# SitaoLuan/When-Do-GNNs-Help

Measured on AMD Instinct MI355X. Metric: aggregation edges/sec (whole job; + %HBM roofline of the SpMM kernel), higher is better.
Workload: dtype f32; 1 GPU; synthetic homophily sweep (data_synthesis/4000-equivalent): 10 h-levels x 5 seeds = 50 graphs/GPU/step, N=2000 nodes, k=10, F=500 fp32, C=5; step = batched D^-1(A+I)X aggregation + edge/label stati...; parallelism=independent sweep shards x1 (no data-path collective; job-table broadcast + r...

## Files before the change

include/wdg.h:

```cpp
#ifndef WDG_H
#define WDG_H

#include <stddef.h>
#include <stdint.h>

#ifdef __cplusplus
extern "C" {
#endif

typedef void *wdg_stream_t;

#define WDG_OK 0
#define WDG_ERR_INVALID (-1)
#define WDG_ERR_LAUNCH (-2)
#define WDG_ERR_WORKSPACE (-3)
#define WDG_ERR_UNSUPPORTED (-4)

int wdg_version(void);
const char *wdg_last_error(void);
int wdg_device_cus(void);

#define WDG_COO_SYMMETRISE 1
#define WDG_COO_BINARISE 2
#define WDG_COO_ADD_SELF_LOOPS 4
// ... 97 lines not shown
    const int32_t *rowptr;
    const int32_t *col;
    const float *val;
    int32_t *q_perm, *q_ext, *q_rows;
    int32_t *q_col;
    float *q_val;
    void *workspace;
    int32_t n_rows, n_cols;
} wdg_sell16_job;
int wdg_csr_to_sell16_count_batched(const wdg_sell16_job *jobs_dev, int32_t n_jobs, int32_t max_rows, int32_t max_cols,
                                    wdg_stream_t stream);
int wdg_csr_to_sell16_fill_batched(const wdg_sell16_job *jobs_dev, int32_t n_jobs, int32_t max_rows, int32_t max_cols,
                                   wdg_stream_t stream);

size_t wdg_csr_band_plan_workspace_bytes(int32_t N);
int32_t wdg_csr_band_perm_len(int32_t N);
int wdg_csr_band_plan(const int32_t *rowptr, int32_t N, int32_t *band_perm, int32_t *band_cuts, void *workspace,
                      size_t workspace_bytes, wdg_stream_t stream);
int wdg_csr_band_plan_hub(const int32_t *rowptr, int32_t N, int32_t hub_len, int32_t *band_perm, int32_t *band_cuts, void *workspace,
                          size_t workspace_bytes, wdg_stream_t stream);

int32_t wdg_spmm_narrow_col_bytes(int32_t n_feat, int32_t x_is_bf16, int32_t has_col_scale);
int32_t wdg_spmm_narrow_parts(int32_t n_cols, int32_t col_bytes);
size_t wdg_spmm_narrow_workspace_bytes(int32_t n_rows, int32_t n_cols);
int wdg_spmm_narrow_plan(const int32_t *rowptr, const int32_t *col, int32_t N, int32_t n_cols, int32_t parts, int32_t *part_ptr,
                         wdg_stream_t stream);
int wdg_spmm_narrow_f32(const wdg_spmm_job *job_host, const int32_t *part_ptr, void *workspace, size_t workspace_bytes,
                        wdg_stream_t stream);
int wdg_spmm_narrow_bf16(const wdg_spmm_job *job_host, const int32_t *part_ptr, void *workspace, size_t workspace_bytes,
                         wdg_stream_t stream);

int wdg_spmm_narrow_batched_f32(const wdg_spmm_job *jobs_dev, int32_t n_jobs, int32_t max_rows, int32_t max_feat, int flags,
                                wdg_stream_t stream);

typedef struct wdg_spmm_item {
    int32_t first_job, n_jobs;
    int32_t unit_begin, unit_end;
    int32_t flags, reserved;
} wdg_spmm_item;
int wdg_spmm_quad_batched_f32(const wdg_spmm_job *jobs_dev, int32_t n_jobs, const wdg_spmm_item *items_dev,
                              const int32_t *seg_ptr_dev, int32_t n_segments, int32_t max_cols, int32_t max_feat, int flags,
                              wdg_stream_t stream);
int wdg_spmm_quad_batched_clocked_f32(const wdg_spmm_job *jobs_dev, int32_t n_jobs, const wdg_spmm_item *items_dev,
                                      const int32_t *seg_ptr_dev, int32_t n_segments, int32_t max_cols, int32_t max_feat,
                                      int flags, uint64_t *wg_clock_dev, wdg_stream_t stream);
int32_t wdg_spmm_quad_workgroups(int32_t n_segments, int32_t max_feat, int flags);
int wdg_debug_clock(uint64_t *out_dev, wdg_stream_t stream);

int wdg_edge_label_stats(const int32_t *rowptr, const int32_t *col, const int32_t *labels, int32_t N, int32_t C,
                         int64_t *totals, int32_t *row_nnz, int32_t *row_nnz_noself, int32_t *row_match_noself,
                         int64_t *compat, int64_t *classdeg, wdg_stream_t stream);

typedef struct wdg_stats_job {
    const int32_t *rowptr;
    const int32_t *col;
    const int32_t *labels;
    int64_t *totals;
    int64_t *compat;
    int64_t *classdeg;
    int32_t *row_nnz, *row_nnz_noself, *row_match_noself;
    int32_t n_rows, n_classes;
} wdg_stats_job;
int wdg_edge_label_stats_batched(const wdg_stats_job *jobs_dev, int32_t n_jobs, int32_t max_rows, int32_t max_classes,
                                 wdg_stream_t stream);

int wdg_sweep_scalars_f32(const int64_t *totals, const int32_t *rows, const int64_t *compat, const int64_t *classdeg,
// ... 207 lines not shown
```

when-do-gnns-help_amd/_lib.py:

```python
import ctypes
import os

os.environ.setdefault("GPU_MAX_HW_QUEUES", "8")

import torch

_HERE = os.path.dirname(os.path.abspath(__file__))
LIB_PATH = os.environ.get("WDG_LIB_PATH") or os.path.join(_HERE, "lib", "libwdg_hip.so")

c_void_p, c_int, c_int32, c_int64, c_size_t = (ctypes.c_void_p, ctypes.c_int, ctypes.c_int32, ctypes.c_int64,
                                               ctypes.c_size_t)
c_uint32 = ctypes.c_uint32


class WdgError(RuntimeError):
    pass


class SpmmJob(ctypes.Structure):
    _fields_ = [("rowptr", c_void_p), ("col", c_void_p), ("val", c_void_p), ("row_scale", c_void_p),
                ("col_scale", c_void_p), ("X", c_void_p), ("Y", c_void_p), ("ldx", c_int64), ("ldy", c_int64),
                ("n_rows", c_int32), ("n_cols", c_int32), ("n_feat", c_int32), ("reserved", c_int32),
                ("q_ext", c_void_p), ("q_col", c_void_p), ("q_val", c_void_p), ("q_perm", c_void_p), ("q_rows", c_void_p),
                ("q_block_cols", c_int32), ("q_n_blocks", c_int32), ("q_n_entries", c_int32), ("q_flags", c_int32),
# ... 30 lines not shown
    "wdg_csr_to_sell16_fill_batched": (c_int, [c_void_p, c_int32, c_int32, c_int32, c_void_p]),
    "wdg_dense_to_csr_count": (c_int, [c_void_p, c_int64, c_int32, c_int32, c_void_p, c_void_p, c_size_t, c_void_p]),
    "wdg_dense_to_csr_fill": (c_int, [c_void_p, c_int64, c_int32, c_int32, c_void_p, c_void_p, c_void_p, c_void_p]),
    "wdg_scan_workspace_bytes": (c_size_t, [c_int64]),
    "wdg_degree_norm": (c_int, [c_void_p, c_void_p, c_int32, c_int, c_int, c_void_p, c_void_p, c_void_p, c_void_p,
                                c_void_p]),
    "wdg_normalise_values": (c_int, [c_void_p, c_void_p, c_void_p, c_int32, c_int, c_int, c_void_p, c_void_p,
                                     c_void_p, c_void_p]),
    "wdg_row_l1_normalise_f32": (c_int, [c_void_p, c_int64, c_void_p, c_int64, c_int32, c_int32, c_int, c_void_p]),
    "wdg_unpack_bits_f32": (c_int, [c_void_p, c_int64, c_int32, c_int32, c_int, c_void_p, c_int64, c_void_p]),
    "wdg_spmm_csr_f32": (c_int, [ctypes.POINTER(SpmmJob), c_void_p]),
    "wdg_spmm_csr_bf16": (c_int, [ctypes.POINTER(SpmmJob), c_void_p]),
    "wdg_spmm_batched_f32": (c_int, [c_void_p, c_int32, c_int32, c_int32, c_int32, c_int, c_void_p]),
    "wdg_spmm_plan": (c_int, [c_int32, c_int32, c_int32, c_int32, c_int, ctypes.POINTER(c_int), ctypes.POINTER(c_int)]),
    "wdg_sell16_block_cols": (c_int32, [c_int32]),
    "wdg_sell16_row_bytes": (c_int32, [c_int32]),
    "wdg_sell16_workspace_bytes": (c_size_t, [c_int32, c_int32]),
    "wdg_sell16_max_entries": (c_int64, [c_int32]),
    "wdg_csr_to_sell16_count": (c_int, [c_void_p, c_void_p, c_int32, c_int32, c_void_p, c_void_p, c_void_p, c_void_p, c_size_t,
                                        c_void_p]),
    "wdg_csr_to_sell16_fill": (c_int, [c_void_p, c_void_p, c_void_p, c_int32, c_int32, c_void_p, c_void_p, c_int32, c_void_p,
                                       c_void_p, c_void_p]),
    "wdg_csr_band_plan_workspace_bytes": (c_size_t, [c_int32]),
    "wdg_csr_band_perm_len": (c_int32, [c_int32]),
    "wdg_csr_band_plan": (c_int, [c_void_p, c_int32, c_void_p, c_void_p, c_void_p, c_size_t, c_void_p]),
    "wdg_csr_band_plan_hub": (c_int, [c_void_p, c_int32, c_int32, c_void_p, c_void_p, c_void_p, c_size_t, c_void_p]),
    "wdg_spmm_narrow_col_bytes": (c_int32, [c_int32, c_int32, c_int32]),
    "wdg_spmm_narrow_parts": (c_int32, [c_int32, c_int32]),
    "wdg_spmm_narrow_workspace_bytes": (c_size_t, [c_int32, c_int32]),
    "wdg_spmm_narrow_plan": (c_int, [c_void_p, c_void_p, c_int32, c_int32, c_int32, c_void_p, c_void_p]),
    "wdg_spmm_narrow_f32": (c_int, [c_void_p, c_void_p, c_void_p, c_size_t, c_void_p]),
    "wdg_spmm_narrow_bf16": (c_int, [c_void_p, c_void_p, c_void_p, c_size_t, c_void_p]),
    "wdg_spmm_narrow_batched_f32": (c_int, [c_void_p, c_int32, c_int32, c_int32, c_int, c_void_p]),
    "wdg_spmm_quad_batched_clocked_f32": (c_int, [c_void_p, c_int32, c_void_p, c_void_p, c_int32, c_int32, c_int32, c_int, c_void_p,
                                                  c_void_p]),
    "wdg_spmm_quad_workgroups": (c_int32, [c_int32, c_int32, c_int]),
    "wdg_debug_clock": (c_int, [c_void_p, c_void_p]),
    "wdg_spmm_quad_batched_f32": (c_int, [c_void_p, c_int32, c_void_p, c_void_p, c_int32, c_int32, c_int32, c_int,
                                          c_void_p]),
    "wdg_edge_label_stats": (c_int, [c_void_p, c_void_p, c_void_p, c_int32, c_int32, c_void_p, c_void_p, c_void_p,
                                     c_void_p, c_void_p, c_void_p, c_void_p]),
    "wdg_edge_label_stats_batched": (c_int, [c_void_p, c_int32, c_int32, c_int32, c_void_p]),
    "wdg_sweep_scalars_f32": (c_int, [c_void_p, c_void_p, c_void_p, c_void_p, c_void_p, c_void_p, c_void_p, c_int32, c_int32, c_int32,
                                      c_void_p, c_void_p]),
    "wdg_edge_cosine_f32": (c_int, [c_void_p, c_void_p, c_void_p, c_int64, c_void_p, c_int64, c_int32, c_int32, c_int,
                                    c_void_p, c_void_p]),
    "wdg_las_workspace_bytes": (c_size_t, [c_int32, c_int32, c_int32]),
    "wdg_las_f32": (c_int, [c_void_p, c_int64, c_void_p, c_void_p, c_int32, c_int32, c_int32, c_void_p, c_void_p,
                            c_void_p, c_size_t, c_void_p]),
    "wdg_gemm_f32": (c_int, [c_void_p, c_int64, c_void_p, c_int64, c_int, c_void_p, c_int, c_void_p, c_int64,
                             c_int32, c_int32, c_int32, c_void_p]),
    "wdg_gemm_skinny_f32": (c_int, [c_void_p, c_int64, c_void_p, c_int64, c_void_p, c_int, c_void_p, c_int64, c_int32, c_int32, c_int32,
                                    c_void_p]),
    "wdg_gemm_splitk_plan": (c_int32, [c_int32, c_int32, c_int32]),
    "wdg_gemm_splitk_workspace_bytes": (c_size_t, [c_int32, c_int32, c_int32]),
    "wdg_gemm_splitk_f32": (c_int, [c_void_p, c_int64, c_void_p, c_int64, c_void_p, c_int, c_void_p, c_int64, c_int32, c_int32, c_int32,
                                    c_int32, c_void_p, c_size_t, c_void_p]),
    "wdg_gemm_batched_f32": (c_int, [c_void_p, c_int32, c_int32, c_int32, c_void_p]),
    "wdg_gemm_batched_flags_f32": (c_int, [c_void_p, c_int32, c_int32, c_int32, c_int32, c_uint32, c_void_p]),
    "wdg_mlp2_batched_f32": (c_int, [c_void_p, c_int32, c_int32, c_int32, c_int32, c_int32, c_void_p]),
    "wdg_mlp2_batched_flags_f32": (c_int, [c_void_p, c_int32, c_int32, c_int32, c_int32, c_int32, c_uint32, c_void_p]),
    "wdg_las_batched_f32": (c_int, [c_void_p, c_int32, c_int32, c_int32, c_int32, c_void_p]),
    "wdg_las_fused_eligible": (c_int, [c_int32, c_int32, c_int32]),
    "wdg_gram_map_batched_f32": (c_int, [c_void_p, c_int32, c_int32, c_void_p]),
    "wdg_gram_map_batched_flags_f32": (c_int, [c_void_p, c_int32, c_int32, c_uint32, c_void_p]),
    "wdg_transpose_batched_f32": (c_int, [c_void_p, c_int32, c_int32, c_int32, c_void_p]),
# ... 116 lines not shown
```

when-do-gnns-help_amd/aggregate.py:

```python
import ctypes
import os

import numpy as np
import torch

from . import _lib
from ._lib import c_void_p, check, lib, require_gpu, stream_handle
from ._rt import *
from ._rt import _dev, _h2d, _ld, _ptr, _table
from ._lib import SpmmItem, SpmmJob
from .graphs import CsrGraph, quad_disabled

ABLATE_BITS = 0


NARROW_MIN_ENTRIES = int(os.environ.get("WDG_NARROW_MIN_ENTRIES", 1 << 15))


def _fill_job(job, g, x, y, row_scale, col_scale, use_values=True, band=False):
    job.rowptr, job.col = g.rowptr.data_ptr(), g.col.data_ptr()
    job.val = g.val.data_ptr() if (use_values and g.val is not None and not g.unit_values) else 0
    job.row_scale = 0 if row_scale is None else row_scale.data_ptr()
    job.col_scale = 0 if col_scale is None else col_scale.data_ptr()
    job.X, job.Y = x.data_ptr(), y.data_ptr()
    if isinstance(y, Tiled):
        if y.cols != x.shape[1] or y.shape[0] != g.n_rows:
            raise ValueError("spmm: a tiled Y must hold exactly the product's rows and columns")
        job.ldx, job.ldy, job.y_group_stride = _ld(x), y.ld, y.group_stride
    else:
        job.ldx, job.ldy, job.y_group_stride = _ld(x), _ld(y), 0
    job.n_rows, job.n_cols, job.n_feat = g.n_rows, g.n_cols, x.shape[1]
    job.reserved = ABLATE_BITS
    wants_val = bool(job.val)
    q = g.quad
    if q and (not wants_val or q["val"] is not None):
        job.q_ext, job.q_col, job.q_perm = q["ext"].data_ptr(), q["col"].data_ptr(), q["perm"].data_ptr()
        job.q_rows = q["rows"].data_ptr()
        job.q_val = q["val"].data_ptr() if (wants_val and q["val"] is not None) else 0
        job.q_block_cols, job.q_n_blocks = q["block_cols"], q["n_blocks"]
        job.q_n_entries, job.q_flags = q["n_entries"], (1 if q["split"] else 0) | (2 if q["half"] else 0) | (4 if isinstance(x, Transposed) else 0)
    else:
        job.q_ext = job.q_col = job.q_val = job.q_perm = job.q_rows = 0
        job.q_block_cols = job.q_n_blocks = job.q_n_entries = job.q_flags = 0
    if band and g.band:
        job.band_perm, job.band_cuts = g.band["perm"].data_ptr(), g.band["cuts"].data_ptr()
        job.band_n_hub = g.band.get("n_hub", -1)
        job.q_ext = job.q_col = job.q_val = job.q_perm = job.q_rows = 0
        job.q_block_cols = job.q_n_blocks = job.q_n_entries = job.q_flags = 0
# ... 217 lines not shown
            if x.dtype != torch.float32 or x.stride(1) != 1:
                raise ValueError("SpmmBatch: X must be fp32 with unit inner stride")
        feats = {e[1].shape[1] for e in entries}
        need_ld = 8 if max(feats, default=0) > 4 else 4
        self.narrow = (len(entries) > 0 and max(feats) <= 8 and os.environ.get("WDG_SPMM_NARROW", "1") != "0"
                       and all(e[1].data_ptr() % 16 == 0 and _ld(e[1]) % 4 == 0 and _ld(e[1]) >= need_ld for e in entries))
        self.quad = (len(entries) > 0 and not self.narrow and not quad_disabled() and min(feats) >= 8
                     and all(e[0].ensure_quad() for e in entries)
                     and all((not (e[5] and e[0].val is not None)) or e[0].quad["val"] is not None for e in entries)
                     and len({e[0].quad["half"] for e in entries}) == 1)
        order = sorted(range(len(entries)), key=lambda i: -entries[i][0].nnz)
        if os.environ.get("WDG_SPMM_ORDER") == "0":
            order = list(range(len(entries)))
        if self.quad:
            groups = _sharing_groups(entries)
            groups.sort(key=lambda grp: -sum(entries[i][0].nnz for i in grp))
            order = [i for grp in groups for i in sorted(grp, key=lambda i: -entries[i][0].nnz)]
        if any(isinstance(e[2], Tiled) for e in entries) and not self.quad:
            raise ValueError("SpmmBatch: a tiled Y needs the quad-row kernel (SELL-16 copies, F >= 8)")
        if any(isinstance(e[1], Transposed) for e in entries) and not self.quad:
            raise ValueError("SpmmBatch: a transposed X needs the quad-row kernel (SELL-16 copies, F >= 8)")
        for job, (g, x, y, rs, cs, uv) in zip(arr, (entries[i] for i in order)):
            _fill_job(job, g, x, y, rs, cs, uv)
            any_val = any_val or bool(job.val)
            dma_ok = dma_ok and _dma_ok(job)
            self.max_rows, self.max_cols = max(self.max_rows, g.n_rows), max(self.max_cols, g.n_cols)
            self.max_feat = max(self.max_feat, x.shape[1])
        self.n_jobs = len(entries)
        self.table = _table(arr)
        self.edges = sum(e[0].nnz for e in entries)
        self.flags = (SPMM_ANY_VAL if any_val else 0) | (SPMM_DMA_OK if dma_ok else 0)
        if any(e[4] is not None for e in entries):
            self.flags |= SPMM_ANY_COL_SCALE
        if self.quad:
            if all(_y_span(e[2], e[0].n_rows) < (1 << 30) and e[0].quad["chunks"] < (1 << 22) - 2 and e[0].quad["split"] for e in entries):
                self.flags |= SPMM_SMALL_OFFSETS
            if entries[0][0].quad["half"]:
                self.flags |= SPMM_HALF_SLAB
            self.order = order
            self._set_segments(None)
            if os.environ.get("WDG_QUAD_VERIFY", "0") not in ("", "0"):
                self.verify()

    def verify(self, tol=1e-5):
        if not self.quad:
            return
        self.launch()
        torch.cuda.synchronize()
        for i, (g, x, y, rs, cs, uv) in enumerate(self.keep):
            got = y.rowmajor() if isinstance(y, Tiled) else y.clone()
            ref = torch.empty((g.n_rows, x.shape[1]), dtype=torch.float32, device=y.device)
            xv = x.t.t().contiguous() if isinstance(x, Transposed) else x
            job = _fill_job(SpmmJob(), g, xv, ref, rs, cs, uv)
            job.q_ext = job.q_col = job.q_val = job.q_perm = job.q_rows = 0
            job.q_block_cols = job.q_n_blocks = job.q_n_entries = job.q_flags = 0
            check(lib.wdg_spmm_csr_f32(ctypes.byref(job), stream_handle()), "wdg_spmm_csr_f32")
            torch.cuda.synchronize()
            err = float((got[:, :x.shape[1]] - ref).abs().max()) if ref.numel() else 0.0
            scale = max(float(ref.abs().max()) if ref.numel() else 0.0, 1e-30)
            if not err <= tol * scale:
                raise RuntimeError(f"WDG_QUAD_VERIFY: job {i} of the quad-row table differs from the CSR kernel by {err:.3e} "
                                   f"(largest entry {scale:.3e})")

    def _set_segments(self, phase_ns, shares=None):
        dev = self.table.device
        items, seg_ptr, self.n_segments = _quad_segments(self.keep, self.order, self.max_feat, max(lib.wdg_device_cus(), 8), phase_ns, shares)
        iarr = (SpmmItem * max(len(items), 1))()
        for it, (fj, nj, ub, ue) in zip(iarr, items):
            it.first_job, it.n_jobs, it.unit_begin, it.unit_end = fj, nj, ub, ue
        self.items = _h2d(torch.frombuffer(bytearray(bytes(iarr)), dtype=torch.uint8), dev)
        self.seg_ptr = _h2d(np.asarray(seg_ptr, np.int32), dev)
        self.n_items = len(items)
        self.items_host, self.seg_ptr_host, self.phase_ns, self.shares = items, seg_ptr, phase_ns, shares

    def segment_spans(self, clock):
# ... 8 lines not shown
            return None
        best = None
        for ph in candidates:
            self._set_segments(ph)
            self.launch()
            e0, e1 = torch.cuda.Event(enable_timing=True), torch.cuda.Event(enable_timing=True)
            torch.cuda.synchronize()
            e0.record()
            for _ in range(launches):
                self.launch()
            e1.record()
            torch.cuda.synchronize()
            t = e0.elapsed_time(e1) / launches
            if best is None or t < best[0]:
                best = (t, ph)
        self._set_segments(best[1])
        self.tuned = best
        return best

    def new_clock(self):
        n = int(lib.wdg_spmm_quad_workgroups(self.n_segments, self.max_feat, self.flags))
        return torch.zeros(2 * n, dtype=torch.int64, device=self.table.device)

    n_launches = 0

    def launch(self, clock=None):
        self.n_launches += 1
        if clock is not None and self.quad:
            check(lib.wdg_spmm_quad_batched_clocked_f32(_ptr(self.table), self.n_jobs, _ptr(self.items), _ptr(self.seg_ptr),
                                                        self.n_segments, self.max_cols, self.max_feat, self.flags, _ptr(clock),
                                                        stream_handle()), "wdg_spmm_quad_batched_clocked_f32")
            return
        if self.narrow:
            check(lib.wdg_spmm_narrow_batched_f32(_ptr(self.table), self.n_jobs, self.max_rows, self.max_feat, self.flags,
                                                  stream_handle()), "wdg_spmm_narrow_batched_f32")
            return
        if self.quad:
            check(lib.wdg_spmm_quad_batched_f32(_ptr(self.table), self.n_jobs, _ptr(self.items), _ptr(self.seg_ptr),
                                                self.n_segments, self.max_cols, self.max_feat, self.flags, stream_handle()),
                  "wdg_spmm_quad_batched_f32")
            return
        check(lib.wdg_spmm_batched_f32(_ptr(self.table), self.n_jobs, self.max_rows, self.max_cols, self.max_feat,
                                       self.flags, stream_handle()), "wdg_spmm_batched_f32")

    def plan(self):
        if self.narrow:
            return 6, 16, 256
        if self.quad:
            return 5, 16, 1024
        return spmm_plan(self.max_rows, self.max_cols, self.max_feat, self.n_jobs, self.flags)

    def kernel_name(self):
        fam, slab, threads = self.plan()
        val = "true" if self.flags & SPMM_ANY_VAL else "false"
        return {0: f"spmm_slab_kernel<{slab},{threads},float>", 1: "spmm_gather_kernel",
                5: f"spmm_quad_kernel<float,{val},{2 if self.flags & SPMM_HALF_SLAB else (1 if self.max_cols > 2528 else 0)}>",
                6: "spmm_narrow_batched_kernel"}.get(fam, f"family {fam}")


def spmm_plan(n_rows, n_cols, n_feat, n_jobs=1, flags=0):
    slab, threads = ctypes.c_int(0), ctypes.c_int(0)
    fam = lib.wdg_spmm_plan(n_jobs, n_rows, n_cols, n_feat, flags, ctypes.byref(slab), ctypes.byref(threads))
    return fam, slab.value, threads.value
```

when-do-gnns-help_amd/csrc/spmm_narrow.hip:

```cpp
#include <algorithm>

#include "wdg_common.h"

namespace {
using namespace wdg;

constexpr int N_THREADS = 256;
constexpr int N_WAVES = N_THREADS / kWave;

typedef unsigned short bf16_t;

template <typename TIN>
__device__ __forceinline__ float n_f32(TIN v);
template <>
__device__ __forceinline__ float n_f32<float>(float v) { return v; }
template <>
__device__ __forceinline__ float n_f32<bf16_t>(bf16_t v) { return __uint_as_float(static_cast<unsigned>(v) << 16); }

template <typename TIN>
__global__ __launch_bounds__(256) void narrow_pack(const TIN *__restrict__ X, int64_t ldx, const float *__restrict__ cs, int n_cols,
                                                   int F, float *__restrict__ T) {
    const int64_t i = static_cast<int64_t>(blockIdx.x) * 256 + threadIdx.x;
    if (i >= static_cast<int64_t>(n_cols) * 8) return;
    const int c = static_cast<int>(i >> 3), f = static_cast<int>(i & 7);
// ... 4 lines not shown

template <typename TIN>
__global__ __launch_bounds__(256) void narrow_pack4(const TIN *__restrict__ X, int64_t ldx, const float *__restrict__ cs, int n_cols,
                                                    int F, float *__restrict__ T) {
    const int64_t i = static_cast<int64_t>(blockIdx.x) * 256 + threadIdx.x;
    if (i >= static_cast<int64_t>(n_cols) * 4) return;
    const int c = static_cast<int>(i >> 2), f = static_cast<int>(i & 3);
    float v = 0.f;
    if (f < F) v = n_f32<TIN>(X[static_cast<int64_t>(c) * ldx + f]) * (cs ? cs[c] : 1.f);
    T[i] = v;
}
__global__ __launch_bounds__(256) void narrow_pack_bf16x8(const bf16_t *__restrict__ X, int64_t ldx, int n_cols, int F,
                                                          bf16_t *__restrict__ T) {
    const int64_t i = static_cast<int64_t>(blockIdx.x) * 256 + threadIdx.x;
    if (i >= static_cast<int64_t>(n_cols) * 8) return;
    const int c = static_cast<int>(i >> 3), f = static_cast<int>(i & 7);
    T[i] = f < F ? X[static_cast<int64_t>(c) * ldx + f] : static_cast<bf16_t>(0);
}

enum { TABLE_F32X8 = 0, TABLE_F32X4 = 1, TABLE_BF16X8 = 2 };

struct Acc8 {
    float v[8];
};

__device__ __forceinline__ void narrow_unpack_bf16(const f32x4_t raw, f32x4_t &lo, f32x4_t &hi) {
    const unsigned w0 = __float_as_uint(raw[0]), w1 = __float_as_uint(raw[1]), w2 = __float_as_uint(raw[2]), w3 = __float_as_uint(raw[3]);
    lo[0] = __uint_as_float(w0 << 16); lo[1] = __uint_as_float(w0 & 0xffff0000u);
    lo[2] = __uint_as_float(w1 << 16); lo[3] = __uint_as_float(w1 & 0xffff0000u);
    hi[0] = __uint_as_float(w2 << 16); hi[1] = __uint_as_float(w2 & 0xffff0000u);
    hi[2] = __uint_as_float(w3 << 16); hi[3] = __uint_as_float(w3 & 0xffff0000u);
}

template <int G, bool HAS_W, bool WIDE = true, bool BF16 = false>
__device__ __forceinline__ Acc8 narrow_sweep(global_ptr<const int32_t> col, global_ptr<const float> val,
                                             global_ptr<const f32x4_t> T, int b, int e, int sub, int64_t ldq = 2,
                                             global_ptr<const float> cs = nullptr) {
    Acc8 a;
#pragma unroll
    for (int f = 0; f < 8; ++f) a.v[f] = 0.f;
    const f32x4_t zero = {0.f, 0.f, 0.f, 0.f};
    int k = b + sub;
    for (; k + 3 * G < e; k += 4 * G) {
        int idx[4];
        float w[4];
        f32x4_t lo[4], hi[4];
#pragma unroll
        for (int u = 0; u < 4; ++u) idx[u] = col[k + u * G];
#pragma unroll
        for (int u = 0; u < 4; ++u) {
            lo[u] = T[ldq * static_cast<int64_t>(idx[u])];
            hi[u] = (WIDE && !BF16) ? T[ldq * static_cast<int64_t>(idx[u]) + 1] : zero;
            w[u] = 1.f;
            if (HAS_W) w[u] = (val ? val[k + u * G] : 1.f) * (cs ? cs[idx[u]] : 1.f);
        }
#pragma unroll
        for (int u = 0; u < 4; ++u) {
            if (BF16) narrow_unpack_bf16(lo[u], lo[u], hi[u]);
#pragma unroll
            for (int f = 0; f < 4; ++f) {
                a.v[f] = HAS_W ? __builtin_fmaf(w[u], lo[u][f], a.v[f]) : a.v[f] + lo[u][f];
                if (WIDE) a.v[4 + f] = HAS_W ? __builtin_fmaf(w[u], hi[u][f], a.v[4 + f]) : a.v[4 + f] + hi[u][f];
            }
        }
    }
    for (; k < e; k += G) {
        const int idx = col[k];
        f32x4_t lo = T[ldq * static_cast<int64_t>(idx)], hi = (WIDE && !BF16) ? T[ldq * static_cast<int64_t>(idx) + 1] : zero;
        if (BF16) narrow_unpack_bf16(lo, lo, hi);
        float w = 1.f;
        if (HAS_W) w = (val ? val[k] : 1.f) * (cs ? cs[idx] : 1.f);
#pragma unroll
        for (int f = 0; f < 4; ++f) {
            a.v[f] = HAS_W ? __builtin_fmaf(w, lo[f], a.v[f]) : a.v[f] + lo[f];
            if (WIDE) a.v[4 + f] = HAS_W ? __builtin_fmaf(w, hi[f], a.v[4 + f]) : a.v[4 + f] + hi[f];
        }
    }
    return a;
}

__device__ __forceinline__ float narrow_reduce16(const Acc8 &a, int lane) {
    float h4[4], h2[2];
    const bool b3 = lane & 8, b2 = lane & 4, b1 = lane & 2;
#pragma unroll
    for (int i = 0; i < 4; ++i) {
        const float keep = b3 ? a.v[4 + i] : a.v[i], send = b3 ? a.v[i] : a.v[4 + i];
        h4[i] = keep + __shfl_xor(send, 8);
    }
#pragma unroll
    for (int i = 0; i < 2; ++i) {
        const float keep = b2 ? h4[2 + i] : h4[i], send = b2 ? h4[i] : h4[2 + i];
        h2[i] = keep + __shfl_xor(send, 4);
    }
    const float keep = b1 ? h2[1] : h2[0], send = b1 ? h2[0] : h2[1];
    const float h1 = keep + __shfl_xor(send, 2);
    return h1 + __shfl_xor(h1, 1);
}

__device__ __forceinline__ float narrow_reduce64(Acc8 a, int lane) {
#pragma unroll
    for (int f = 0; f < 8; ++f) a.v[f] += __shfl_xor(a.v[f], 32);
// ... 65 lines not shown
        int b = 0, e = 0;
        if (live) bounds(row, b, e);
        const float total = narrow_reduce16(narrow_sweep<16, HAS_VAL, WIDE, BF16>(col, val, T, b, e, lane & 15, LDQ), lane);
        if (live && !(lane & 1) && feat < n_out) out[static_cast<int64_t>(row) * ldo + feat] = total * scale_of(row);
    }
}

__global__ __launch_bounds__(256) void narrow_plan_kernel(const int32_t *__restrict__ rowptr, const int32_t *__restrict__ col, int N,
                                                          int part_cols, int parts, int32_t *__restrict__ part_ptr) {
    const int64_t i = static_cast<int64_t>(blockIdx.x) * 256 + threadIdx.x;
    if (i >= static_cast<int64_t>(N) * (parts - 1)) return;
    const int row = static_cast<int>(i / (parts - 1)), p = static_cast<int>(i % (parts - 1)) + 1;
    int lo = rowptr[row], hi = rowptr[row + 1];
    const int key = p * part_cols;
    while (lo < hi) {
        const int mid = (lo + hi) >> 1;
        if (col[mid] < key) lo = mid + 1;
        else hi = mid;
    }
    part_ptr[i] = lo;
}

__global__ __launch_bounds__(256) void narrow_combine(const float *__restrict__ P, int N, int parts, int F, const float *__restrict__ rs,
                                                      float *__restrict__ Y, int64_t ldy) {
    const int64_t i = static_cast<int64_t>(blockIdx.x) * 256 + threadIdx.x;
    if (i >= static_cast<int64_t>(N) * 8) return;
    const int row = static_cast<int>(i >> 3), f = static_cast<int>(i & 7);
    if (f >= F) return;
    float sum = P[i];
    for (int p = 1; p < parts; ++p) sum += P[static_cast<int64_t>(p) * N * 8 + i];
    Y[static_cast<int64_t>(row) * ldy + f] = sum * (rs ? rs[row] : 1.f);
}

template <bool HAS_W, bool WIDE>
__global__ __launch_bounds__(N_THREADS) void spmm_narrow_batched_kernel(const wdg_spmm_job *__restrict__ jobs, int blocks_per_job) {
    const int job_id = blockIdx.x / blocks_per_job, rb = blockIdx.x % blocks_per_job;
    const desc_ptr<wdg_spmm_job> job = (desc_ptr<wdg_spmm_job>)(jobs + job_id);
    const int N = job->n_rows, F = job->n_feat;
    const int lane = threadIdx.x & 63;
    const int row = rb * 16 + (threadIdx.x >> 4);
    if (rb * 16 >= N) return;
    const global_ptr<const int32_t> rowptr = to_global(job->rowptr), col = to_global(job->col);
    const global_ptr<const float> val = to_global(job->val), rs = to_global(job->row_scale), cs = to_global(job->col_scale);
    const global_ptr<const f32x4_t> X = (global_ptr<const f32x4_t>)to_global(static_cast<const float *>(job->X));
    const bool live = row < N;
    const int b = live ? rowptr[row] : 0, e = live ? rowptr[row + 1] : 0;
    const float total = narrow_reduce16(narrow_sweep<16, HAS_W, WIDE>(col, val, X, b, e, lane & 15, job->ldx / 4, cs), lane);
    const int feat = (lane >> 1) & 7;
    if (live && !(lane & 1) && feat < F) to_global(job->Y)[static_cast<int64_t>(row) * job->ldy + feat] = total * (rs ? rs[row] : 1.f);
}

constexpr int64_t N_PART_BYTES = 3 << 20;

}

extern "C" {

int32_t wdg_spmm_narrow_col_bytes(int32_t n_feat, int32_t x_is_bf16, int32_t has_col_scale) {
    return (n_feat <= 4 || (x_is_bf16 && !has_col_scale)) ? 16 : 32;
}

int32_t wdg_spmm_narrow_parts(int32_t n_cols, int32_t col_bytes) {
    if (const char *s = getenv("WDG_NARROW_PARTS")) {
        const int v = atoi(s);
        if (v == 1 || v == 2 || v == 4 || v == 8) return v;
    }
    int parts = 1;
    while (parts < 8 && static_cast<int64_t>(n_cols) * col_bytes > N_PART_BYTES * parts) parts <<= 1;
    return parts;
}

size_t wdg_spmm_narrow_workspace_bytes(int32_t n_rows, int32_t n_cols) {
    const int parts = wdg_spmm_narrow_parts(n_cols, 32);
    return static_cast<size_t>(n_cols > 0 ? n_cols : 0) * 32 + (parts > 1 ? static_cast<size_t>(parts) * (n_rows > 0 ? n_rows : 0) * 32 : 0) + 512;
}

int wdg_spmm_narrow_plan(const int32_t *rowptr, const int32_t *col, int32_t N, int32_t n_cols, int32_t parts, int32_t *part_ptr,
                         wdg_stream_t stream) {
    WDG_REQUIRE(N >= 0 && n_cols >= 0, "spmm_narrow_plan: negative size");
    WDG_REQUIRE(parts == 1 || parts == 2 || parts == 4 || parts == 8, "spmm_narrow_plan: parts must be 1, 2, 4 or 8");
    if (parts == 1 || N == 0) return WDG_OK;
    WDG_REQUIRE(rowptr && col && part_ptr, "spmm_narrow_plan: null array");
// ... 37 lines not shown
        else
            hipLaunchKernelGGL(narrow_pack<float>, dim3(blocks), dim3(256), 0, st, static_cast<const float *>(j->X), j->ldx, j->col_scale, j->n_cols, j->n_feat, T);
    }
    const int cus = std::max(wdg_device_cus(), 8);
    const int per_cu = 8;
    const dim3 grid(static_cast<unsigned>(cus / kXcds * kXcds * per_cu));
#define WDG_NARROW_LAUNCH(V, TB) hipLaunchKernelGGL((spmm_narrow_kernel<V, TB>), grid, dim3(N_THREADS), 0, st, *j, T, part_ptr, parts, P)
    if (j->val) {
        if (table == TABLE_F32X8) WDG_NARROW_LAUNCH(true, TABLE_F32X8);
        else if (table == TABLE_F32X4) WDG_NARROW_LAUNCH(true, TABLE_F32X4);
        else WDG_NARROW_LAUNCH(true, TABLE_BF16X8);
    } else {
        if (table == TABLE_F32X8) WDG_NARROW_LAUNCH(false, TABLE_F32X8);
        else if (table == TABLE_F32X4) WDG_NARROW_LAUNCH(false, TABLE_F32X4);
        else WDG_NARROW_LAUNCH(false, TABLE_BF16X8);
    }
#undef WDG_NARROW_LAUNCH
    if (parts > 1) {
        const unsigned blocks = static_cast<unsigned>(wdg::ceil_div(static_cast<int64_t>(j->n_rows) * 8, 256));
        hipLaunchKernelGGL(narrow_combine, dim3(blocks), dim3(256), 0, st, P, j->n_rows, parts, j->n_feat, j->row_scale, j->Y, j->ldy);
    }
    return wdg::check_launch("spmm_narrow_kernel");
}

int wdg_spmm_narrow_f32(const wdg_spmm_job *job_host, const int32_t *part_ptr, void *workspace, size_t workspace_bytes,
                        wdg_stream_t stream) {
    return narrow_launch(job_host, false, part_ptr, workspace, workspace_bytes, stream);
}
int wdg_spmm_narrow_bf16(const wdg_spmm_job *job_host, const int32_t *part_ptr, void *workspace, size_t workspace_bytes,
                         wdg_stream_t stream) {
    return narrow_launch(job_host, true, part_ptr, workspace, workspace_bytes, stream);
}

int wdg_spmm_narrow_batched_f32(const wdg_spmm_job *jobs_dev, int32_t n_jobs, int32_t max_rows, int32_t max_feat, int flags,
                                wdg_stream_t stream) {
    WDG_REQUIRE(n_jobs >= 0 && max_rows >= 0 && max_feat >= 0, "spmm_narrow_batched: negative size");
    if (n_jobs == 0 || max_rows == 0 || max_feat == 0) return WDG_OK;
    WDG_REQUIRE(jobs_dev != nullptr, "spmm_narrow_batched: null job table");
    if (max_feat > 8) return wdg::fail(WDG_ERR_UNSUPPORTED, "spmm_narrow_batched: more than 8 features");
    const int blocks_per_job = static_cast<int>(wdg::ceil_div(max_rows, 16));
    WDG_REQUIRE(static_cast<int64_t>(blocks_per_job) * n_jobs < (1ll << 31), "spmm_narrow_batched: grid too large");
    const dim3 grid(static_cast<unsigned>(blocks_per_job) * n_jobs);
    hipStream_t st = wdg::as_stream(stream);
    const bool has_w = (flags & (WDG_SPMM_ANY_VAL | WDG_SPMM_ANY_COL_SCALE)) != 0, wide = max_feat > 4;
    if (has_w) {
        if (wide) hipLaunchKernelGGL((spmm_narrow_batched_kernel<true, true>), grid, dim3(N_THREADS), 0, st, jobs_dev, blocks_per_job);
        else hipLaunchKernelGGL((spmm_narrow_batched_kernel<true, false>), grid, dim3(N_THREADS), 0, st, jobs_dev, blocks_per_job);
    } else {
        if (wide) hipLaunchKernelGGL((spmm_narrow_batched_kernel<false, true>), grid, dim3(N_THREADS), 0, st, jobs_dev, blocks_per_job);
        else hipLaunchKernelGGL((spmm_narrow_batched_kernel<false, false>), grid, dim3(N_THREADS), 0, st, jobs_dev, blocks_per_job);
    }
    return wdg::check_launch("spmm_narrow_batched_kernel");
}

}
```

when-do-gnns-help_amd/ops.py:

```python
from ._lib import check, lib, require_gpu, stream_handle
from ._rt import (
    ACT_NONE, ACT_RELU, COO_ADD_SELF_LOOPS, COO_BINARISE, COO_DROP_SELF_LOOPS, COO_KEEP_DUPLICATES, COO_SYMMETRISE,
    GEMM_A_VEC4, NORM_RW, NORM_SYM, PREC_F32, PREC_F64, SPMM_ANY_COL_SCALE, SPMM_ANY_VAL, SPMM_DMA_OK,
    SPMM_HALF_SLAB, SPMM_SMALL_OFFSETS, Tiled, Transposed, _dev, _h2d, _H2D_MAX_BYTES, _ld, _PinnedArena, _ptr, _table,
)
from .graphs import (
    CsrGraph, degree_norm, GraphBatch, normalise_values, quad_disabled, row_l1_normalise, unpack_bits,
    _host_pack_coo,
)
from .aggregate import (
    QUAD_MULTI_ITEM_SU, spmm, spmm_plan, SpmmBatch, _dma_ok, _fill_job, _QUAD_COST_NS,
    _QUAD_COST_W, _quad_cut, _quad_segments, _quad_unit_cost, _quad_unit_costs, _sharing_groups,
)
from .stats import (
    edge_cosine, edge_label_stats, las, LasBatch, StatsBatch,
)
from .gemm import (
    gemm, gemm_skinny, GemmBatch, Mlp2Batch,
)
from .kernel_regression import (
    deflation_enabled, EdgeGramBatch, GnbBatch, GramBatch, kr_split_sizes, KrBatch, KrSets, PropagatedGram, RowRepBatch, SvmBatch, _KR_JOB_DTYPE,
)
```

Measured before the change: 18.16 billion edges/s.

## Stage narrow SpMM source rows in LDS with software-pipelined row extents

Adds an LDS-staged route for the batched narrow SpMM. Each workgroup of 512 threads copies the whole narrow source matrix (and column scales) of its job into up to 128 KiB of dynamic LDS, then sweeps a contiguous slice of rows. It also prefetches row extents and the first four column indices two steps ahead. The host chooses a parts-per-job count from CU count, rows and the edge-to-column ratio. This replaces scattered global gathers with LDS reads, at the cost of a redundant per-workgroup staging load and occupancy limited to one large block per CU.

```diff
diff --git a/include/wdg.h b/include/wdg.h
--- a/include/wdg.h
+++ b/include/wdg.h
@@ -153,6 +153,12 @@
 
 int wdg_spmm_narrow_batched_f32(const wdg_spmm_job *jobs_dev, int32_t n_jobs, int32_t max_rows, int32_t max_feat, int flags,
                                 wdg_stream_t stream);
+#define WDG_NARROW_IN_PLACE 0
+#define WDG_NARROW_LDS_512 1
+#define WDG_NARROW_LDS_1024 2
+int32_t wdg_spmm_narrow_lds_bytes(int32_t max_cols, int32_t max_feat, int flags);
+int wdg_spmm_narrow_batched_routed_f32(const wdg_spmm_job *jobs_dev, int32_t n_jobs, int32_t max_rows, int32_t max_cols,
+                                       int32_t max_feat, int flags, int32_t route, int32_t parts, wdg_stream_t stream);
 
 typedef struct wdg_spmm_item {
     int32_t first_job, n_jobs;
diff --git a/when-do-gnns-help_amd/_lib.py b/when-do-gnns-help_amd/_lib.py
--- a/when-do-gnns-help_amd/_lib.py
+++ b/when-do-gnns-help_amd/_lib.py
@@ -86,6 +86,8 @@
     "wdg_spmm_narrow_f32": (c_int, [c_void_p, c_void_p, c_void_p, c_size_t, c_void_p]),
     "wdg_spmm_narrow_bf16": (c_int, [c_void_p, c_void_p, c_void_p, c_size_t, c_void_p]),
     "wdg_spmm_narrow_batched_f32": (c_int, [c_void_p, c_int32, c_int32, c_int32, c_int, c_void_p]),
+    "wdg_spmm_narrow_lds_bytes": (c_int32, [c_int32, c_int32, c_int]),
+    "wdg_spmm_narrow_batched_routed_f32": (c_int, [c_void_p, c_int32, c_int32, c_int32, c_int32, c_int, c_int32, c_int32, c_void_p]),
     "wdg_spmm_quad_batched_clocked_f32": (c_int, [c_void_p, c_int32, c_void_p, c_void_p, c_int32, c_int32, c_int32, c_int, c_void_p,
                                                   c_void_p]),
     "wdg_spmm_quad_workgroups": (c_int32, [c_int32, c_int32, c_int]),
diff --git a/when-do-gnns-help_amd/aggregate.py b/when-do-gnns-help_amd/aggregate.py
--- a/when-do-gnns-help_amd/aggregate.py
+++ b/when-do-gnns-help_amd/aggregate.py
@@ -14,6 +14,9 @@
 ABLATE_BITS = 0
 
 
+NARROW_IN_PLACE, NARROW_LDS_512, NARROW_LDS_1024 = 0, 1, 2
+NARROW_LDS_SHAPE = (512, NARROW_LDS_512)
+NARROW_LDS_FACTOR = 2
 NARROW_MIN_ENTRIES = int(os.environ.get("WDG_NARROW_MIN_ENTRIES", 1 << 15))
 
 
@@ -297,6 +300,7 @@
         self.flags = (SPMM_ANY_VAL if any_val else 0) | (SPMM_DMA_OK if dma_ok else 0)
         if any(e[4] is not None for e in entries):
             self.flags |= SPMM_ANY_COL_SCALE
+        self.narrow_route, self.narrow_parts = self._narrow_route(entries) if self.narrow else (NARROW_IN_PLACE, 1)
         if self.quad:
             if all(_y_span(e[2], e[0].n_rows) < (1 << 30) and e[0].quad["chunks"] < (1 << 22) - 2 and e[0].quad["split"] for e in entries):
                 self.flags |= SPMM_SMALL_OFFSETS
@@ -306,6 +310,18 @@
             self._set_segments(None)
             if os.environ.get("WDG_QUAD_VERIFY", "0") not in ("", "0"):
                 self.verify()
+
+    def _narrow_route(self, entries):
+        threads, route = NARROW_LDS_SHAPE
+        if os.environ.get("WDG_NARROW_LDS", "1") == "0" or lib.wdg_spmm_narrow_lds_bytes(self.max_cols, self.max_feat, self.flags) < 0:
+            return NARROW_IN_PLACE, 1
+        staged = sum(e[0].n_cols for e in entries)
+        parts = min(max(2 * max(lib.wdg_device_cus(), 8) // len(entries), 1), -(-self.max_rows // (threads // 16)),
+                    int(self.edges // (NARROW_LDS_FACTOR * staged)) if staged else 1)
+        if os.environ.get("WDG_NARROW_LDS_SHAPE"):
+            t, parts = (int(v) for v in os.environ["WDG_NARROW_LDS_SHAPE"].split("x"))
+            route = {512: NARROW_LDS_512, 1024: NARROW_LDS_1024}[t]
+        return (route, parts) if parts >= 1 else (NARROW_IN_PLACE, 1)
 
     def verify(self, tol=1e-5):
         if not self.quad:
@@ -380,8 +396,9 @@
                                                         stream_handle()), "wdg_spmm_quad_batched_clocked_f32")
             return
         if self.narrow:
-            check(lib.wdg_spmm_narrow_batched_f32(_ptr(self.table), self.n_jobs, self.max_rows, self.max_feat, self.flags,
-                                                  stream_handle()), "wdg_spmm_narrow_batched_f32")
+            check(lib.wdg_spmm_narrow_batched_routed_f32(_ptr(self.table), self.n_jobs, self.max_rows, self.max_cols, self.max_feat,
+                                                         self.flags, self.narrow_route, self.narrow_parts, stream_handle()),
+                  "wdg_spmm_narrow_batched_routed_f32")
             return
         if self.quad:
             check(lib.wdg_spmm_quad_batched_f32(_ptr(self.table), self.n_jobs, _ptr(self.items), _ptr(self.seg_ptr),
diff --git a/when-do-gnns-help_amd/csrc/spmm_narrow.hip b/when-do-gnns-help_amd/csrc/spmm_narrow.hip
--- a/when-do-gnns-help_amd/csrc/spmm_narrow.hip
+++ b/when-do-gnns-help_amd/csrc/spmm_narrow.hip
@@ -60,15 +60,56 @@
     hi[2] = __uint_as_float(w3 << 16); hi[3] = __uint_as_float(w3 & 0xffff0000u);
 }
 
-template <int G, bool HAS_W, bool WIDE = true, bool BF16 = false>
-__device__ __forceinline__ Acc8 narrow_sweep(global_ptr<const int32_t> col, global_ptr<const float> val,
-                                             global_ptr<const f32x4_t> T, int b, int e, int sub, int64_t ldq = 2,
-                                             global_ptr<const float> cs = nullptr) {
+struct First4 {
+    int idx[4];
+    float val[4];
+};
+template <int G>
+__device__ __forceinline__ First4 narrow_first4(global_ptr<const int32_t> col, global_ptr<const float> val, int b, int e, int sub) {
+    First4 p;
+#pragma unroll
+    for (int u = 0; u < 4; ++u) {
+        const int k = b + sub + u * G;
+        p.idx[u] = k < e ? col[k] : 0;
+        p.val[u] = (val && k < e) ? val[k] : 1.f;
+    }
+    return p;
+}
+
+template <int G, bool HAS_W, bool WIDE = true, bool BF16 = false, typename TP = global_ptr<const f32x4_t>,
+          typename CP = global_ptr<const float>, bool PRE = false>
+__device__ __forceinline__ Acc8 narrow_sweep(global_ptr<const int32_t> col, global_ptr<const float> val, TP T, int b, int e, int sub,
+                                             int64_t ldq = 2, CP cs = nullptr, int64_t hiq = 1, const First4 &first = First4{}) {
     Acc8 a;
 #pragma unroll
     for (int f = 0; f < 8; ++f) a.v[f] = 0.f;
     const f32x4_t zero = {0.f, 0.f, 0.f, 0.f};
     int k = b + sub;
+    if constexpr (PRE) {
+        float w[4];
+        f32x4_t lo[4], hi[4];
+#pragma unroll
+        for (int u = 0; u < 4; ++u) {
+            if (k + u * G < e) {
+                lo[u] = T[ldq * static_cast<int64_t>(first.idx[u])];
+                hi[u] = (WIDE && !BF16) ? T[ldq * static_cast<int64_t>(first.idx[u]) + hiq] : zero;
+                w[u] = 1.f;
+                if (HAS_W) w[u] = first.val[u] * (cs ? cs[first.idx[u]] : 1.f);
+            }
+        }
+#pragma unroll
+        for (int u = 0; u < 4; ++u) {
+            if (k + u * G < e) {
+                if (BF16) narrow_unpack_bf16(lo[u], lo[u], hi[u]);
+#pragma unroll
+                for (int f = 0; f < 4; ++f) {
+                    a.v[f] = HAS_W ? __builtin_fmaf(w[u], lo[u][f], a.v[f]) : a.v[f] + lo[u][f];
+                    if (WIDE) a.v[4 + f] = HAS_W ? __builtin_fmaf(w[u], hi[u][f], a.v[4 + f]) : a.v[4 + f] + hi[u][f];
+                }
+            }
+        }
+        k += 4 * G;
+    }
     for (; k + 3 * G < e; k += 4 * G) {
         int idx[4];
         float w[4];
@@ -78,7 +119,7 @@
 #pragma unroll
         for (int u = 0; u < 4; ++u) {
             lo[u] = T[ldq * static_cast<int64_t>(idx[u])];
-            hi[u] = (WIDE && !BF16) ? T[ldq * static_cast<int64_t>(idx[u]) + 1] : zero;
+            hi[u] = (WIDE && !BF16) ? T[ldq * static_cast<int64_t>(idx[u]) + hiq] : zero;
             w[u] = 1.f;
             if (HAS_W) w[u] = (val ? val[k + u * G] : 1.f) * (cs ? cs[idx[u]] : 1.f);
         }
@@ -94,7 +135,7 @@
     }
     for (; k < e; k += G) {
         const int idx = col[k];
-        f32x4_t lo = T[ldq * static_cast<int64_t>(idx)], hi = (WIDE && !BF16) ? T[ldq * static_cast<int64_t>(idx) + 1] : zero;
+        f32x4_t lo = T[ldq * static_cast<int64_t>(idx)], hi = (WIDE && !BF16) ? T[ldq * static_cast<int64_t>(idx) + hiq] : zero;
         if (BF16) narrow_unpack_bf16(lo, lo, hi);
         float w = 1.f;
         if (HAS_W) w = (val ? val[k] : 1.f) * (cs ? cs[idx] : 1.f);
@@ -226,22 +267,87 @@
     Y[static_cast<int64_t>(row) * ldy + f] = sum * (rs ? rs[row] : 1.f);
 }
 
-template <bool HAS_W, bool WIDE>
-__global__ __launch_bounds__(N_THREADS) void spmm_narrow_batched_kernel(const wdg_spmm_job *__restrict__ jobs, int blocks_per_job) {
-    const int job_id = blockIdx.x / blocks_per_job, rb = blockIdx.x % blocks_per_job;
+template <typename T>
+using lds_ptr = T __attribute__((address_space(3))) *;
+
+constexpr int N_LDS_CAP = 128 * 1024;
+
+extern __shared__ __attribute__((aligned(16))) f32x4_t narrow_slab[];
+
+template <bool HAS_W, bool WIDE, int LDS_THREADS = 0>
+__global__ __launch_bounds__(LDS_THREADS ? LDS_THREADS : N_THREADS, 1) void spmm_narrow_batched_kernel(const wdg_spmm_job *__restrict__ jobs, int per_job) {
+    const int job_id = blockIdx.x / per_job, rb = blockIdx.x % per_job;
     const desc_ptr<wdg_spmm_job> job = (desc_ptr<wdg_spmm_job>)(jobs + job_id);
     const int N = job->n_rows, F = job->n_feat;
     const int lane = threadIdx.x & 63;
-    const int row = rb * 16 + (threadIdx.x >> 4);
-    if (rb * 16 >= N) return;
+    const int feat = (lane >> 1) & 7;
     const global_ptr<const int32_t> rowptr = to_global(job->rowptr), col = to_global(job->col);
     const global_ptr<const float> val = to_global(job->val), rs = to_global(job->row_scale), cs = to_global(job->col_scale);
     const global_ptr<const f32x4_t> X = (global_ptr<const f32x4_t>)to_global(static_cast<const float *>(job->X));
-    const bool live = row < N;
-    const int b = live ? rowptr[row] : 0, e = live ? rowptr[row + 1] : 0;
-    const float total = narrow_reduce16(narrow_sweep<16, HAS_W, WIDE>(col, val, X, b, e, lane & 15, job->ldx / 4, cs), lane);
-    const int feat = (lane >> 1) & 7;
-    if (live && !(lane & 1) && feat < F) to_global(job->Y)[static_cast<int64_t>(row) * job->ldy + feat] = total * (rs ? rs[row] : 1.f);
+    const global_ptr<float> Y = to_global(job->Y);
+    if constexpr (LDS_THREADS == 0) {
+        const int row = rb * 16 + (threadIdx.x >> 4);
+        if (rb * 16 >= N) return;
+        const bool live = row < N;
+        const int b = live ? rowptr[row] : 0, e = live ? rowptr[row + 1] : 0;
+        const float total = narrow_reduce16(narrow_sweep<16, HAS_W, WIDE>(col, val, X, b, e, lane & 15, job->ldx / 4, cs), lane);
+        if (live && !(lane & 1) && feat < F) Y[static_cast<int64_t>(row) * job->ldy + feat] = total * (rs ? rs[row] : 1.f);
+    } else {
+        constexpr int WAVES = LDS_THREADS / kWave;
+        const int part_rows = ((N + 15) / 16 + per_job - 1) / per_job * 16;
+        const int row0 = rb * part_rows;
+        if (row0 >= N) return;
+        const int row_end = min(row0 + part_rows, N), n_cols = job->n_cols;
+        const int tid = threadIdx.x, wave = tid >> 6;
+        auto extent = [&](int row, int &b, int &e, float &scale) {
+            const int r = min(row, row_end - 1);
+            b = rowptr[r], e = rowptr[r + 1];
+            scale = rs ? rs[r] : 1.f;
+            if (row >= row_end) e = b;
+        };
+        constexpr int STEP = 4 * WAVES;
+        int row = row0 + wave * 4 + (lane >> 4), b, e, b1, e1;
+        float scale, scale1;
+        extent(row, b, e, scale);
+        extent(row + STEP, b1, e1, scale1);
+        First4 first = narrow_first4<16>(col, val, b, e, lane & 15);
+        const lds_ptr<f32x4_t> slab = (lds_ptr<f32x4_t>)narrow_slab;
+        const lds_ptr<float> slab_cs = (lds_ptr<float>)(slab + (WIDE ? 2 : 1) * n_cols);
+        const int64_t ldq = job->ldx / 4;
+        const int n_quads = (WIDE ? 2 : 1) * n_cols;
+        for (int i0 = tid; i0 < n_quads; i0 += 4 * LDS_THREADS) {
+            f32x4_t v[4];
+#pragma unroll
+            for (int u = 0; u < 4; ++u) {
+                const int i = i0 + u * LDS_THREADS, c = WIDE ? i >> 1 : i, h = WIDE ? i & 1 : 0;
+                if (i < n_quads) v[u] = X[ldq * c + h];
+            }
+#pragma unroll
+            for (int u = 0; u < 4; ++u) {
+                const int i = i0 + u * LDS_THREADS, c = WIDE ? i >> 1 : i, h = WIDE ? i & 1 : 0;
+                if (i < n_quads) slab[h * n_cols + c] = v[u];
+            }
+        }
+        const bool has_cs = HAS_W && cs;
+        if (has_cs)
+            for (int i = tid; i < n_cols; i += LDS_THREADS) slab_cs[i] = cs[i];
+        __syncthreads();
+        const lds_ptr<const f32x4_t> T = (lds_ptr<const f32x4_t>)slab;
+        const lds_ptr<const float> lcs = has_cs ? (lds_ptr<const float>)slab_cs : nullptr;
+        const int64_t ldy = job->ldy;
+        for (; row - (lane >> 4) < row_end; row += STEP) {
+            int b2, e2;
+            float scale2;
+            extent(row + 2 * STEP, b2, e2, scale2);
+            const First4 first1 = narrow_first4<16>(col, val, b1, e1, lane & 15);
+            const Acc8 acc = narrow_sweep<16, HAS_W, WIDE, false, lds_ptr<const f32x4_t>, lds_ptr<const float>, true>(col, val, T, b, e, lane & 15,
+                                                                                                                     1, lcs, n_cols, first);
+            const float total = narrow_reduce16(acc, lane);
+            if (row < row_end && !(lane & 1) && feat < F) Y[static_cast<int64_t>(row) * ldy + feat] = total * scale;
+            b = b1, e = e1, scale = scale1, first = first1;
+            b1 = b2, e1 = e2, scale1 = scale2;
+        }
+    }
 }
 
 constexpr int64_t N_PART_BYTES = 3 << 20;
@@ -345,25 +451,57 @@
     return narrow_launch(job_host, true, part_ptr, workspace, workspace_bytes, stream);
 }
 
-int wdg_spmm_narrow_batched_f32(const wdg_spmm_job *jobs_dev, int32_t n_jobs, int32_t max_rows, int32_t max_feat, int flags,
-                                wdg_stream_t stream) {
-    WDG_REQUIRE(n_jobs >= 0 && max_rows >= 0 && max_feat >= 0, "spmm_narrow_batched: negative size");
+int32_t wdg_spmm_narrow_lds_bytes(int32_t max_cols, int32_t max_feat, int flags) {
+    if (max_cols < 0 || max_feat < 0 || max_feat > 8) return -1;
+    const int64_t bytes = static_cast<int64_t>(max_cols) * ((max_feat > 4 ? 32 : 16) + ((flags & WDG_SPMM_ANY_COL_SCALE) ? 4 : 0));
+    return bytes <= N_LDS_CAP ? static_cast<int32_t>(bytes) : -1;
+}
+
+int wdg_spmm_narrow_batched_routed_f32(const wdg_spmm_job *jobs_dev, int32_t n_jobs, int32_t max_rows, int32_t max_cols, int32_t max_feat,
+                                       int flags, int32_t route, int32_t parts, wdg_stream_t stream) {
+    WDG_REQUIRE(n_jobs >= 0 && max_rows >= 0 && max_cols >= 0 && max_feat >= 0, "spmm_narrow_batched: negative size");
+    WDG_REQUIRE(route == WDG_NARROW_IN_PLACE || route == WDG_NARROW_LDS_512 || route == WDG_NARROW_LDS_1024, "spmm_narrow_batched: unknown route");
     if (n_jobs == 0 || max_rows == 0 || max_feat == 0) return WDG_OK;
     WDG_REQUIRE(jobs_dev != nullptr, "spmm_narrow_batched: null job table");
     if (max_feat > 8) return wdg::fail(WDG_ERR_UNSUPPORTED, "spmm_narrow_batched: more than 8 features");
-    const int blocks_per_job = static_cast<int>(wdg::ceil_div(max_rows, 16));
-    WDG_REQUIRE(static_cast<int64_t>(blocks_per_job) * n_jobs < (1ll << 31), "spmm_narrow_batched: grid too large");
-    const dim3 grid(static_cast<unsigned>(blocks_per_job) * n_jobs);
     hipStream_t st = wdg::as_stream(stream);
     const bool has_w = (flags & (WDG_SPMM_ANY_VAL | WDG_SPMM_ANY_COL_SCALE)) != 0, wide = max_feat > 4;
-    if (has_w) {
-        if (wide) hipLaunchKernelGGL((spmm_narrow_batched_kernel<true, true>), grid, dim3(N_THREADS), 0, st, jobs_dev, blocks_per_job);
-        else hipLaunchKernelGGL((spmm_narrow_batched_kernel<true, false>), grid, dim3(N_THREADS), 0, st, jobs_dev, blocks_per_job);
-    } else {
-        if (wide) hipLaunchKernelGGL((spmm_narrow_batched_kernel<false, true>), grid, dim3(N_THREADS), 0, st, jobs_dev, blocks_per_job);
-        else hipLaunchKernelGGL((spmm_narrow_batched_kernel<false, false>), grid, dim3(N_THREADS), 0, st, jobs_dev, blocks_per_job);
-    }
+#define WDG_NARROW_BATCHED(T, PER_JOB, THREADS, LDS)                                                                             \
+    do {                                                                                                                         \
+        const dim3 grid(static_cast<unsigned>(PER_JOB) * n_jobs);                                                                \
+        if (has_w && wide) hipLaunchKernelGGL((spmm_narrow_batched_kernel<true, true, T>), grid, dim3(THREADS), LDS, st, jobs_dev, PER_JOB);        \
+        else if (has_w) hipLaunchKernelGGL((spmm_narrow_batched_kernel<true, false, T>), grid, dim3(THREADS), LDS, st, jobs_dev, PER_JOB);         \
+        else if (wide) hipLaunchKernelGGL((spmm_narrow_batched_kernel<false, true, T>), grid, dim3(THREADS), LDS, st, jobs_dev, PER_JOB);          \
+        else hipLaunchKernelGGL((spmm_narrow_batched_kernel<false, false, T>), grid, dim3(THREADS), LDS, st, jobs_dev, PER_JOB);                   \
+    } while (0)
+    if (route == WDG_NARROW_IN_PLACE) {
+        const int blocks_per_job = static_cast<int>(wdg::ceil_div(max_rows, 16));
+        WDG_REQUIRE(static_cast<int64_t>(blocks_per_job) * n_jobs < (1ll << 31), "spmm_narrow_batched: grid too large");
+        WDG_NARROW_BATCHED(0, blocks_per_job, N_THREADS, 0);
+        return wdg::check_launch("spmm_narrow_batched_kernel");
+    }
+    const int lds = wdg_spmm_narrow_lds_bytes(max_cols, max_feat, flags);
+    if (lds < 0) return wdg::fail(WDG_ERR_UNSUPPORTED, "spmm_narrow_batched: the LDS route needs every job's sources within 128 KiB");
+    WDG_REQUIRE(parts >= 1 && static_cast<int64_t>(parts) * n_jobs < (1ll << 31), "spmm_narrow_batched: parts out of range");
+    static thread_local int configured_dev = -1;
+    if (configured_dev != wdg::current_device()) {
+        for (const void *k : {reinterpret_cast<const void *>(spmm_narrow_batched_kernel<true, true, 512>), reinterpret_cast<const void *>(spmm_narrow_batched_kernel<true, false, 512>),
+                              reinterpret_cast<const void *>(spmm_narrow_batched_kernel<false, true, 512>), reinterpret_cast<const void *>(spmm_narrow_batched_kernel<false, false, 512>),
+                              reinterpret_cast<const void *>(spmm_narrow_batched_kernel<true, true, 1024>), reinterpret_cast<const void *>(spmm_narrow_batched_kernel<true, false, 1024>),
+                              reinterpret_cast<const void *>(spmm_narrow_batched_kernel<false, true, 1024>), reinterpret_cast<const void *>(spmm_narrow_batched_kernel<false, false, 1024>)})
+            if (hipFuncSetAttribute(k, hipFuncAttributeMaxDynamicSharedMemorySize, N_LDS_CAP) != hipSuccess)
+                return wdg::fail(WDG_ERR_LAUNCH, "hipFuncSetAttribute(max dynamic LDS) failed");
+        configured_dev = wdg::current_device();
+    }
+    if (route == WDG_NARROW_LDS_512) WDG_NARROW_BATCHED(512, parts, 512, static_cast<size_t>(lds));
+    else WDG_NARROW_BATCHED(1024, parts, 1024, static_cast<size_t>(lds));
+#undef WDG_NARROW_BATCHED
     return wdg::check_launch("spmm_narrow_batched_kernel");
 }
 
-}
+int wdg_spmm_narrow_batched_f32(const wdg_spmm_job *jobs_dev, int32_t n_jobs, int32_t max_rows, int32_t max_feat, int flags,
+                                wdg_stream_t stream) {
+    return wdg_spmm_narrow_batched_routed_f32(jobs_dev, n_jobs, max_rows, 0, max_feat, flags, WDG_NARROW_IN_PLACE, 1, stream);
+}
+
+}
diff --git a/when-do-gnns-help_amd/ops.py b/when-do-gnns-help_amd/ops.py
--- a/when-do-gnns-help_amd/ops.py
+++ b/when-do-gnns-help_amd/ops.py
@@ -9,7 +9,7 @@
     _host_pack_coo,
 )
 from .aggregate import (
-    QUAD_MULTI_ITEM_SU, spmm, spmm_plan, SpmmBatch, _dma_ok, _fill_job, _QUAD_COST_NS,
+    NARROW_IN_PLACE, NARROW_LDS_512, NARROW_LDS_1024, QUAD_MULTI_ITEM_SU, spmm, spmm_plan, SpmmBatch, _dma_ok, _fill_job, _QUAD_COST_NS,
     _QUAD_COST_W, _quad_cut, _quad_segments, _quad_unit_cost, _quad_unit_costs, _sharing_groups,
 )
 from .stats import (
```

Result: faster. 18.43 billion edges/s, median of 5 (+1.5%).
